# LLaVA-VL/LLaVA-Plus-Codebase

Hardware: NVIDIA H100
Metric: prefill+decode tokens/s (higher is better)
Workload: dtype bf16

## Files before the change

llava-plus-codebase_b200/csrc/decode_mega.cu:

```cuda
#include <limits.h>
#include <math.h>

#include "common.cuh"
#include "kernels.h"

namespace b2 {
namespace {

constexpr int MK_CONS_WARPS = 16;
constexpr int MK_CONS = MK_CONS_WARPS * 32;
constexpr int MK_PROD_WARPS = 4;
constexpr int MK_THREADS = MK_CONS + 32 * MK_PROD_WARPS;
constexpr int MK_D = 128;
constexpr int MK_U = 4;
constexpr int MK_KT = 2048;
constexpr int MK_ROW_PAD = 64;
constexpr int MK_ROW_STRIDE = MK_KT * 2 + MK_ROW_PAD;
constexpr int MK_TILE_BYTES = 8 * MK_ROW_STRIDE;
constexpr int MK_MAXNB = 32;
constexpr int MK_MAXL = 48;
constexpr int MK_MAX_STAGES = 12;

__device__ __forceinline__ void unpack8(const uint4& u, float (&f)[8]) {
    f[0] = bf16_lo(u.x); f[1] = bf16_hi(u.x); f[2] = bf16_lo(u.y); f[3] = bf16_hi(u.y);
    f[4] = bf16_lo(u.z); f[5] = bf16_hi(u.z); f[6] = bf16_lo(u.w); f[7] = bf16_hi(u.w);
}
__device__ __forceinline__ uint4 ldcg16(const void* p) { return __ldcg(reinterpret_cast<const uint4*>(p)); }

__device__ __forceinline__ void cons_sync() { asm volatile("bar.sync 1, %0;" ::"n"(MK_CONS) : "memory"); }

__device__ __forceinline__ void grid_sync(unsigned int* counter, unsigned int target) {
    cons_sync();
    if (threadIdx.x == 0) {
        asm volatile("red.release.gpu.global.add.u32 [%0], 1;" ::"l"(counter) : "memory");
        unsigned int cur, spins = 0;
        do {
            asm volatile("ld.acquire.gpu.global.u32 %0, [%1];" : "=r"(cur) : "l"(counter) : "memory");
            if (++spins > (1u << 26)) asm volatile("trap;");
        } while ((int)(cur - target) < 0);
    }
    cons_sync();
}

__device__ __forceinline__ void bulk_g2s(void* smem_dst, const void* gsrc, uint32_t bytes, uint64_t* bar) {
    asm volatile("cp.async.bulk.shared::cluster.global.mbarrier::complete_tx::bytes [%0], [%1], %2, [%3];" ::"r"(
                     smem_u32(smem_dst)),
                 "l"(gsrc), "r"(bytes), "r"(smem_u32(bar))
                 : "memory");
}

struct GemvCtx {
    const __nv_bfloat16* W;
    int K, act;
    int u_lo, nu;
    int nb;
    int nchunk;
};
struct PhaseIO {
    const __nv_bfloat16* xin;
    const __nv_bfloat16* gamma;
    const __nv_bfloat16* residual;
    void* out;
    int ld_out, out_fp32;
};

__device__ __forceinline__ int mk_phys_row(const GemvCtx& c, int rb, int g, bool& valid) {
    if (c.act == ACT_SWIGLU) {
        const int lc = rb * 4 + (g & 3);
        valid = lc < c.nu;
        const int ch = c.u_lo + lc;
        return (ch >> 6) * 128 + (ch & 63) + ((g >> 2) ? 64 : 0);
    }
    const int lr = rb * 8 + g;
    valid = lr < c.nu;
    return c.u_lo + lr;
}

__device__ __forceinline__ int mk_rows_in_block(const GemvCtx& c, int rb) {
    if (c.act == ACT_SWIGLU) return 2 * min(4, c.nu - rb * 4);
    return min(8, c.nu - rb * 8);
}

__device__ __forceinline__ bool mk_is_attention(const MegaParams& p, int ph) { return ph % 5 == 1 && ph < 5 * p.L; }

__device__ __forceinline__ PhaseIO mk_phase_io(const MegaParams& p, const MegaLayer* layers, int ph) {
    PhaseIO c;
    const int l = ph / 5, k = ph % 5;
    c.gamma = nullptr; c.residual = nullptr; c.out_fp32 = 0;
    if (l >= p.L) { c.xin = p.x; c.gamma = p.final_norm; c.out = p.logits; c.ld_out = p.V; c.out_fp32 = 1; }
    else if (k <= 1) { c.xin = p.x; c.gamma = layers[l].ln1; c.out = p.qkv; c.ld_out = 3 * p.h; }
    else if (k == 2) { c.xin = p.attn; c.residual = p.x; c.out = p.x; c.ld_out = p.h; }
    else if (k == 3) { c.xin = p.x; c.gamma = layers[l].ln2; c.out = p.act; c.ld_out = p.I; }
    else { c.xin = p.act; c.residual = p.x; c.out = p.x; c.ld_out = p.h; }
    return c;
}
__device__ __forceinline__ GemvCtx mk_phase_ctx(const MegaParams& p, const MegaLayer* layers, int ph) {
    GemvCtx c;
    const int l = ph / 5, k = ph % 5;
    int N;
    c.act = ACT_NONE;
    if (l >= p.L) { c.W = p.lm_head; N = p.V; c.K = p.h; }
    else if (k <= 1) { c.W = layers[l].wqkv; N = 3 * p.h; c.K = p.h; }
    else if (k == 2) { c.W = layers[l].wo; N = p.h; c.K = p.h; }
    else if (k == 3) { c.W = layers[l].wgu; N = 2 * p.I; c.K = p.h; c.act = ACT_SWIGLU; }
    else { c.W = layers[l].wd; N = p.h; c.K = p.I; }
    const long long units = c.act == ACT_SWIGLU ? (N >> 1) : N;
    c.u_lo = (int)((units * blockIdx.x) / gridDim.x);
    c.nu = (int)((units * (blockIdx.x + 1)) / gridDim.x) - c.u_lo;
    c.nb = c.act == ACT_SWIGLU ? (c.nu + 3) >> 2 : (c.nu + 7) >> 3;
    c.nchunk = (c.K + MK_KT - 1) / MK_KT;
    return c;
}

template <int NB>
__device__ __forceinline__ void mk_prologue(const PhaseIO& c, int K, int B, float eps, int tid, int lane, int warp,
                                            __nv_bfloat16* xs, float (*s_red)[NB], float* s_rstd,
                                            const __nv_bfloat16* gamma_smem) {
    const int nvec = K >> 3;
    float ss[NB];
#pragma unroll
    for (int b = 0; b < NB; ++b) ss[b] = 0.f;
    for (int i = tid; i < nvec; i += MK_CONS) {
#pragma unroll
        for (int b = 0; b < NB; ++b) {
            uint4 u = make_uint4(0, 0, 0, 0);
            if (b < B) u = ldcg16(c.xin + (size_t)b * K + i * 8);
            *reinterpret_cast<uint4*>(xs + (size_t)b * K + i * 8) = u;
            if (c.gamma != nullptr) {
                float f[8];
                unpack8(u, f);
#pragma unroll
                for (int e = 0; e < 8; ++e) ss[b] += f[e] * f[e];
            }
        }
    }
    if (c.gamma != nullptr) {
// ... 22 lines not shown
                const float rstd = s_rstd[b];
#pragma unroll
                for (int e = 0; e < 8; ++e) o[e] = gf[e] * round_bf16(f[e] * rstd);
                *px = make_uint4(pack_bf16(o[0], o[1]), pack_bf16(o[2], o[3]), pack_bf16(o[4], o[5]),
                                 pack_bf16(o[6], o[7]));
            }
        }
    }
    cons_sync();
}

__device__ __forceinline__ void mk_mma(float (&c)[4], uint32_t a0, uint32_t a2, uint32_t b0, uint32_t b1) {
    asm volatile(
        "mma.sync.aligned.m16n8k16.row.col.f32.bf16.bf16.f32 {%0,%1,%2,%3}, {%4,%5,%6,%7}, {%8,%9}, {%0,%1,%2,%3};"
        : "+f"(c[0]), "+f"(c[1]), "+f"(c[2]), "+f"(c[3])
        : "r"(a0), "r"(0u), "r"(a2), "r"(0u), "r"(b0), "r"(b1));
}

template <int NB>
__device__ __forceinline__ float mk_row_value(const float* s_gpart, int rb, int b, int r) {
    float v = 0.f;
#pragma unroll
    for (int ww = 0; ww < MK_CONS_WARPS; ++ww) v += s_gpart[(((size_t)ww * MK_MAXNB + rb) * NB + b) * 8 + r];
    return v;
}

template <int NB>
__device__ __forceinline__ void mk_epilogue(const MegaParams& p, const MegaLayer* layers, int ph, const GemvCtx& c,
                                            int B, int tid, const float* s_gpart, float res_pref, bool have_res_pref) {
    const PhaseIO io = mk_phase_io(p, layers, ph);
    if (c.act == ACT_SWIGLU) {
        const int nch = c.nu;
        for (int idx = tid; idx < nch * B; idx += MK_CONS) {
            const int b = idx / nch, r = idx - b * nch;
            const int rb = r >> 2, q = r & 3;
            const float gt = mk_row_value<NB>(s_gpart, rb, b, q);
            const float up = mk_row_value<NB>(s_gpart, rb, b, q + 4);
            reinterpret_cast<__nv_bfloat16*>(io.out)[(size_t)b * io.ld_out + (size_t)c.u_lo + r] =
                __float2bfloat16_rn(gt / (1.0f + __expf(-gt)) * up);
        }
    } else {
        const int nr = c.nu;
        for (int idx = tid; idx < nr * B; idx += MK_CONS) {
            const int b = idx / nr, r = idx - b * nr;
            float y = mk_row_value<NB>(s_gpart, r >> 3, b, r & 7);
            const size_t o = (size_t)b * io.ld_out + (size_t)c.u_lo + r;
            if (io.residual != nullptr) y += have_res_pref ? res_pref : __bfloat162float(__ldcg(io.residual + o));
            if (io.out_fp32) reinterpret_cast<float*>(io.out)[o] = y;
            else reinterpret_cast<__nv_bfloat16*>(io.out)[o] = __float2bfloat16_rn(y);
        }
    }
}

__device__ __forceinline__ void mk_attention(const MegaParams& p, const MegaLayer& Lw, int tid, int lane, int warp,
                                             float (*s_part)[MK_D + 2], int* s_flag, const float* s_cos,
                                             const float* s_sin) {
    const int h = p.h, H = p.H;
    const int pairs = p.B * H;
    const int grid = gridDim.x;
    const int G = pairs <= grid ? grid / pairs : 1;
    const int hw = lane >> 4, c = lane & 15;
    const int split = pairs <= grid ? (int)blockIdx.x % G : 0;
    for (int pair = pairs <= grid ? (int)blockIdx.x / G : (int)blockIdx.x; pair < pairs;
         pair += (pairs <= grid ? pairs : grid)) {
        const int head = pair % H, b = pair / H;
        const int pos = p.cur_len[b];
        const int total = pos + 1;
        const int cchunk = (total + G - 1) / G;
        const int cb = split * cchunk;
        const int ce = min(cb + cchunk, total);
        const int wchunk = (max(ce - cb, 0) + MK_CONS_WARPS - 1) / MK_CONS_WARPS;
        const int k_begin = cb + warp * wchunk;
        const int k_end = min(k_begin + wchunk, ce);
        const __nv_bfloat16* qrow = p.qkv + (size_t)b * 3 * h + head * MK_D;
        float qreg[8], knew[8], vnew[8];
        {
            float qa[8], qb[8], ka[8], kb[8];
            unpack8(ldcg16(qrow + c * 8), qa);
            unpack8(ldcg16(qrow + (c ^ 8) * 8), qb);
            unpack8(ldcg16(qrow + h + c * 8), ka);
            unpack8(ldcg16(qrow + h + (c ^ 8) * 8), kb);
            unpack8(ldcg16(qrow + 2 * h + c * 8), vnew);
            const float sign = (c < 8) ? -1.f : 1.f;
#pragma unroll
            for (int e = 0; e < 8; ++e) {
                const int i = ((c & 7) * 8 + e);
                const float cbf = s_cos[b * 64 + i], sbf = s_sin[b * 64 + i];
                qreg[e] = round_bf16(round_bf16(qa[e] * cbf) + round_bf16(sign * qb[e] * sbf));
                knew[e] = round_bf16(round_bf16(ka[e] * cbf) + round_bf16(sign * kb[e] * sbf));
            }
        }
        const size_t cbase = ((size_t)b * H + head) * p.Smax * MK_D;
        if (pos >= k_begin && pos < k_end && hw == 0) {
            *reinterpret_cast<uint4*>(Lw.kcache + cbase + (size_t)pos * MK_D + c * 8) =
                make_uint4(pack_bf16(knew[0], knew[1]), pack_bf16(knew[2], knew[3]),
                           pack_bf16(knew[4], knew[5]), pack_bf16(knew[6], knew[7]));
            *reinterpret_cast<uint4*>(Lw.vcache + cbase + (size_t)pos * MK_D + c * 8) =
                make_uint4(pack_bf16(vnew[0], vnew[1]), pack_bf16(vnew[2], vnew[3]),
                           pack_bf16(vnew[4], vnew[5]), pack_bf16(vnew[6], vnew[7]));
        }
        float m_run = -INFINITY, l_run = 0.f, av[8];
#pragma unroll
        for (int e = 0; e < 8; ++e) av[e] = 0.f;
        const __nv_bfloat16* kb_ = Lw.kcache + cbase + c * 8;
        const __nv_bfloat16* vb_ = Lw.vcache + cbase + c * 8;
        for (int kbase = k_begin; kbase < k_end; kbase += 2 * MK_U) {
            uint4 kraw[MK_U], vraw[MK_U];
#pragma unroll
            for (int u = 0; u < MK_U; ++u) {
                const int key = kbase + hw + 2 * u;
                if (key < k_end && key != pos) {
                    kraw[u] = ld_stream_16(kb_ + (size_t)key * MK_D);
                    vraw[u] = ld_stream_16(vb_ + (size_t)key * MK_D);
                } else {
                    kraw[u] = make_uint4(0, 0, 0, 0);
                    vraw[u] = make_uint4(0, 0, 0, 0);
                }
            }
#pragma unroll
            for (int u = 0; u < MK_U; ++u) {
                const int key = kbase + hw + 2 * u;
                float kf[8], vf[8];
                unpack8(kraw[u], kf);
                unpack8(vraw[u], vf);
                if (key == pos) {
#pragma unroll
                    for (int e = 0; e < 8; ++e) { kf[e] = knew[e]; vf[e] = vnew[e]; }
// ... 30 lines not shown
            }
            l_run = l_run * w_s + l_o * w_o;
            m_run = m_c;
        }
        if (hw == 0) {
#pragma unroll
            for (int e = 0; e < 8; ++e) s_part[warp][c * 8 + e] = av[e];
            if (c == 0) { s_part[warp][MK_D] = m_run; s_part[warp][MK_D + 1] = l_run; }
        }
        cons_sync();
        float m_cta = -INFINITY, l_cta = 0.f, o_cta = 0.f;
        if (tid < MK_D) {
#pragma unroll
            for (int i = 0; i < MK_CONS_WARPS; ++i) m_cta = fmaxf(m_cta, s_part[i][MK_D]);
#pragma unroll
            for (int i = 0; i < MK_CONS_WARPS; ++i) {
                const float ms = s_part[i][MK_D];
                const float wgt = (ms == -INFINITY) ? 0.f : exp2f(ms - m_cta);
                l_cta += s_part[i][MK_D + 1] * wgt;
                o_cta += s_part[i][tid] * wgt;
            }
        }
        if (G == 1) {
            if (tid < MK_D) p.attn[(size_t)b * h + head * MK_D + tid] = __float2bfloat16_rn(o_cta / l_cta);
        } else {
            float* part = p.attn_partial + ((size_t)pair * G + split) * (MK_D + 2);
            if (tid < MK_D) {
                part[tid] = o_cta;
                if (tid == 0) { part[MK_D] = m_cta; part[MK_D + 1] = l_cta; }
            }
            __threadfence();
            cons_sync();
            if (tid == 0) *s_flag = (atomicAdd(&p.attn_counters[pair], 1) == G - 1) ? 1 : 0;
            cons_sync();
            if (*s_flag) {
                __threadfence();
                if (tid < MK_D) {
                    const float* pb = p.attn_partial + (size_t)pair * G * (MK_D + 2);
                    float m_all = -INFINITY;
                    for (int sidx = 0; sidx < G; ++sidx) m_all = fmaxf(m_all, __ldcg(pb + (size_t)sidx * (MK_D + 2) + MK_D));
                    float l_all = 0.f, o_all = 0.f;
                    for (int sidx = 0; sidx < G; ++sidx) {
                        const float ms = __ldcg(pb + (size_t)sidx * (MK_D + 2) + MK_D);
                        const float wgt = (ms == -INFINITY) ? 0.f : exp2f(ms - m_all);
                        l_all += __ldcg(pb + (size_t)sidx * (MK_D + 2) + MK_D + 1) * wgt;
                        o_all += __ldcg(pb + (size_t)sidx * (MK_D + 2) + tid) * wgt;
                    }
                    p.attn[(size_t)b * h + head * MK_D + tid] = __float2bfloat16_rn(o_all / l_all);
                    if (tid == 0) p.attn_counters[pair] = 0;
                }
            }
        }
        cons_sync();
    }
}

struct TileCursor {
    GemvCtx c;
    int ph, rb, kc;
    uint32_t tile;
    bool valid;
};
__device__ __forceinline__ void cursor_seek(TileCursor& t, const MegaParams& p, const MegaLayer* layers, int n_phases) {
    while (t.ph < n_phases) {
        if (!mk_is_attention(p, t.ph)) {
            t.c = mk_phase_ctx(p, layers, t.ph);
            if (t.c.nb > 0) { t.rb = 0; t.kc = 0; t.valid = true; return; }
        }
        ++t.ph;
    }
    t.valid = false;
}
__device__ __forceinline__ void cursor_begin(TileCursor& t, const MegaParams& p, const MegaLayer* layers, int n_phases) {
    t.ph = 0; t.tile = 0; t.rb = 0; t.kc = 0;
    cursor_seek(t, p, layers, n_phases);
}
__device__ __forceinline__ void cursor_next(TileCursor& t, const MegaParams& p, const MegaLayer* layers, int n_phases) {
    ++t.tile;
    if (++t.kc < t.c.nchunk) return;
    t.kc = 0;
    if (++t.rb < t.c.nb) return;
    ++t.ph;
    cursor_seek(t, p, layers, n_phases);
}
template <int NB>
__global__ void __launch_bounds__(MK_THREADS, 1) decode_mega_kernel(MegaParams p, int n_stages) {
    extern __shared__ __align__(128) uint8_t mk_smem[];
    uint8_t* ring = mk_smem;
    __nv_bfloat16* xs = reinterpret_cast<__nv_bfloat16*>(ring + (size_t)n_stages * MK_TILE_BYTES);
    float* s_gpart = reinterpret_cast<float*>(reinterpret_cast<uint8_t*>(xs) + (size_t)NB * (p.h > p.I ? p.h : p.I) * 2);
    uint64_t* full_bar = reinterpret_cast<uint64_t*>(s_gpart + (size_t)MK_CONS_WARPS * MK_MAXNB * NB * 8);
    uint64_t* empty_bar = full_bar + MK_MAX_STAGES;
    __shared__ float s_red[MK_CONS_WARPS][NB];
    __shared__ float s_rstd[NB];
    __shared__ float s_av[MK_CONS_WARPS];
    __shared__ int s_ai[MK_CONS_WARPS];
    __shared__ float s_part[MK_CONS_WARPS][MK_D + 2];
    __shared__ int s_flag;
    __shared__ float s_cos[NB * 64], s_sin[NB * 64];
    __shared__ __align__(16) MegaLayer s_layers[MK_MAXL];

    const int tid = threadIdx.x, lane = tid & 31, warp = tid >> 5;
    const int B = p.B;
    const int n_phases = 5 * p.L + 1;

    {
// ... 12 lines not shown

    if (warp >= MK_CONS_WARPS) {
        const uint32_t pw = (uint32_t)(warp - MK_CONS_WARPS);
        TileCursor cp;
        cursor_begin(cp, p, s_layers, n_phases);
        while (cp.valid) {
            if (cp.tile % (uint32_t)MK_PROD_WARPS == pw) {
                const uint32_t stage = cp.tile % (uint32_t)n_stages;
                const uint32_t parity = (cp.tile / (uint32_t)n_stages) & 1u;
                const uint32_t row_bytes = (uint32_t)min(MK_KT, cp.c.K - cp.kc * MK_KT) * 2u;
                if (lane == 0) {
                    mbar_wait(&empty_bar[stage], parity ^ 1u);
                    mbar_arrive_expect_tx(&full_bar[stage], (uint32_t)mk_rows_in_block(cp.c, cp.rb) * row_bytes);
                }
                __syncwarp();
                bool row_valid;
                const int prow = mk_phys_row(cp.c, cp.rb, lane & 7, row_valid);
                if (lane < 8 && row_valid)
                    bulk_g2s(ring + (size_t)stage * MK_TILE_BYTES + (size_t)lane * MK_ROW_STRIDE,
                             cp.c.W + (size_t)prow * cp.c.K + (size_t)cp.kc * MK_KT, row_bytes, &full_bar[stage]);
            }
            cursor_next(cp, p, s_layers, n_phases);
        }
        return;
    }

    for (int i = tid; i < B * 64; i += MK_CONS) {
        const int b = i >> 6, f = i & 63;
        const float inv_freq = exp2f(-(2.0f * f / MK_D) * log2f(p.theta));
        float sv, cv;
        sincosf((float)p.cur_len[b] * inv_freq, &sv, &cv);
        s_cos[i] = round_bf16(cv);
        s_sin[i] = round_bf16(sv);
    }
    if (blockIdx.x < B) {
        int t = p.tok[blockIdx.x];
        t = t < 0 ? 0 : (t >= p.V ? p.V - 1 : t);
        const uint4* src = reinterpret_cast<const uint4*>(p.embed + (size_t)t * p.h);
        uint4* dst = reinterpret_cast<uint4*>(p.x + (size_t)blockIdx.x * p.h);
        for (int i = tid; i < p.h / 8; i += MK_CONS) dst[i] = src[i];
    }
    __nv_bfloat16* gsm = xs + (size_t)NB * p.h;
    const bool gsm_fits = (size_t)(NB + 1) * p.h <= (size_t)NB * (p.h > p.I ? p.h : p.I);
    auto gamma_prefetch = [&](int ph) -> bool {
        if (!gsm_fits || ph >= n_phases || mk_is_attention(p, ph)) return false;
        const PhaseIO io = mk_phase_io(p, s_layers, ph);
        if (io.gamma == nullptr) return false;
        for (int i = tid; i < (p.h >> 3); i += MK_CONS)
            asm volatile("cp.async.cg.shared.global [%0], [%1], 16;" ::"r"(smem_u32(gsm + i * 8)), "l"(io.gamma + i * 8) : "memory");
        asm volatile("cp.async.commit_group;" ::: "memory");
        return true;
    };
    bool gsm_ok = gamma_prefetch(0);
    unsigned int bar_target = p.bar_base + gridDim.x;
    grid_sync(p.bar_count, bar_target);

    const bool tracing = p.trace != nullptr && blockIdx.x == 0 && tid == 0;
    const int g = lane >> 2, t4 = lane & 3;
    uint32_t tile = 0;
#pragma unroll 1
    for (int ph = 0; ph < n_phases; ++ph) {
        if (tracing) p.trace[ph * 4 + 0] = clock64();
        if (mk_is_attention(p, ph)) {
            mk_attention(p, s_layers[ph / 5], tid, lane, warp, s_part, &s_flag, s_cos, s_sin);
        } else {
            const GemvCtx c = mk_phase_ctx(p, s_layers, ph);
            const PhaseIO io = mk_phase_io(p, s_layers, ph);
            const bool have_res = io.residual != nullptr && c.nu * B <= MK_CONS;
            float res_pref = 0.f;
            if (have_res && tid < c.nu * B) {
                const int b = tid / c.nu, r = tid - b * c.nu;
                res_pref = __bfloat162float(__ldcg(io.residual + (size_t)b * io.ld_out + (size_t)c.u_lo + r));
            }
            mk_prologue<NB>(io, c.K, B, p.eps, tid, lane, warp, xs, s_red, s_rstd, gsm_ok ? gsm : nullptr);
            if (tracing) p.trace[ph * 4 + 1] = clock64();
#pragma unroll 1
            for (int rb = 0; rb < c.nb; ++rb) {
                float acc[4] = {0.f, 0.f, 0.f, 0.f}, acc2[4] = {0.f, 0.f, 0.f, 0.f};
#pragma unroll 1
                for (int kc = 0; kc < c.nchunk; ++kc, ++tile) {
                    const uint32_t stage = tile % (uint32_t)n_stages;
                    const uint32_t parity = (tile / (uint32_t)n_stages) & 1u;
                    const int nk32 = min(MK_KT, c.K - kc * MK_KT) >> 5;
                    mbar_wait(&full_bar[stage], parity);
                    const uint8_t* trow = ring + (size_t)stage * MK_TILE_BYTES + (size_t)g * MK_ROW_STRIDE + t4 * 16;
                    const __nv_bfloat16* xrow = xs + (size_t)g * c.K + (size_t)kc * MK_KT + t4 * 8;
#pragma unroll 4
                    for (int k32 = warp; k32 < nk32; k32 += MK_CONS_WARPS) {
                        const uint4 wv = *reinterpret_cast<const uint4*>(trow + k32 * 64);
                        uint4 xv = make_uint4(0, 0, 0, 0);
                        if (g < B) xv = *reinterpret_cast<const uint4*>(xrow + k32 * 32);
                        mk_mma(acc, xv.x, xv.y, wv.x, wv.y);
                        mk_mma(acc2, xv.z, xv.w, wv.z, wv.w);
                    }
                    __syncwarp();
                    if (lane == 0) mbar_arrive(&empty_bar[stage]);
                }
                if (g < NB)
                    *reinterpret_cast<float2*>(s_gpart + (((size_t)warp * MK_MAXNB + rb) * NB + g) * 8 + t4 * 2) =
                        make_float2(acc[0] + acc2[0], acc[1] + acc2[1]);
            }
            cons_sync();
            if (tracing) p.trace[ph * 4 + 2] = clock64();
            mk_epilogue<NB>(p, s_layers, ph, c, B, tid, s_gpart, res_pref, have_res);
        }
        if (tracing) p.trace[ph * 4 + 3] = clock64();
        gsm_ok = gamma_prefetch(ph + 1);
        bar_target += gridDim.x;
        grid_sync(p.bar_count, bar_target);
    }
    if (tracing) p.trace[n_phases * 4] = clock64();

    if (blockIdx.x < B) {
        const int b = blockIdx.x;
        const float* row = p.logits + (size_t)b * p.V;
        float best = -INFINITY;
        int bi = INT_MAX;
        for (int i = tid; i < p.V; i += MK_CONS) {
            const float v = __ldcg(row + i);
            if (v == v && (bi == INT_MAX || v > best)) { best = v; bi = i; }
        }
#pragma unroll
        for (int o = 16; o > 0; o >>= 1) {
            const float ov = __shfl_xor_sync(0xffffffffu, best, o);
            const int oi = __shfl_xor_sync(0xffffffffu, bi, o);
            if (ov > best || (ov == best && oi < bi)) { best = ov; bi = oi; }
        }
        if (lane == 0) { s_av[warp] = best; s_ai[warp] = bi; }
        cons_sync();
        if (warp == 0) {
            best = lane < MK_CONS_WARPS ? s_av[lane] : -INFINITY;
            bi = lane < MK_CONS_WARPS ? s_ai[lane] : INT_MAX;
#pragma unroll
            for (int o = 16; o > 0; o >>= 1) {
                const float ov = __shfl_xor_sync(0xffffffffu, best, o);
                const int oi = __shfl_xor_sync(0xffffffffu, bi, o);
                if (ov > best || (ov == best && oi < bi)) { best = ov; bi = oi; }
            }
            if (lane == 0) {
                const int tk = bi == INT_MAX ? 0 : bi;
                p.tok[b] = tk;
                p.out_tokens[(size_t)(*p.step_counter) * B + b] = tk;
                if (p.rows == nullptr || p.rows[b].active) p.cur_len[b] += 1;
                if (p.ring != nullptr) {
                    const int pub = p.sstate->pub_counter, tag0 = p.sstate->tag;
                    if (tag0 != 0) {
                        const int tag = 1 + (tag0 - 1 + pub / p.ring_cap) % 2047;
                        reinterpret_cast<volatile int32_t*>(p.ring)[(size_t)(pub % p.ring_cap) * B + b] = (tag << 20) | (tk & 0xFFFFF);
                        __threadfence_system();
                    }
                }
            }
        }
    }
    cons_sync();
    if (tid == 0) {
        __threadfence();
        if (atomicAdd(p.done_count, 1u) == gridDim.x - 1) {
            *p.done_count = 0u;
            *p.step_counter += 1;
            if (p.ring != nullptr) p.sstate->pub_counter += 1;
        }
    }
}

size_t mega_fixed_bytes(int NB, int h, int I) {
    return (size_t)NB * (h > I ? h : I) * 2 + (size_t)MK_CONS_WARPS * MK_MAXNB * NB * 8 * 4 + 2 * MK_MAX_STAGES * 8;
}
size_t mega_static_bytes(int NB) {
    return (size_t)(MK_CONS_WARPS + 1) * NB * 4 + MK_CONS_WARPS * (MK_D + 2 + 2) * 4 + NB * 512 +
           MK_MAXL * sizeof(MegaLayer) + 1024;
}
int mega_stages(int NB, int h, int I) {
    const long long avail = 227 * 1024 - (long long)mega_fixed_bytes(NB, h, I) - (long long)mega_static_bytes(NB);
    long long s = avail / MK_TILE_BYTES;
    return (int)(s > MK_MAX_STAGES ? MK_MAX_STAGES : s);
}

}

bool decode_mega_fits(int B, int h, int I) {
    if (B < 1 || B > 2) return false;
    return mega_stages(B, h, I) >= 4;
}

int decode_mega(const MegaParams& p, cudaStream_t stream) {
    B2_CHECK_ARG(p.B >= 1 && p.B <= 2, "decode_mega: batch must be 1..2");
    B2_CHECK_ARG(p.L <= MK_MAXL, "decode_mega: %d layers exceed the shared layer table (%d)", p.L, MK_MAXL);
    B2_CHECK_ARG(p.h % 256 == 0 && p.I % 256 == 0 && p.V % 8 == 0 && p.h / p.H == MK_D,
                 "decode_mega: unsupported dims h=%d I=%d V=%d H=%d", p.h, p.I, p.V, p.H);
    {
        const int grid = num_sms();
        const int nmax = p.V > 3 * p.h ? (p.V > 2 * p.I ? p.V : 2 * p.I) : (3 * p.h > 2 * p.I ? 3 * p.h : 2 * p.I);
        B2_CHECK_ARG((nmax / 8 + grid - 1) / grid + 1 <= MK_MAXNB,
                     "decode_mega: %d output rows per CTA exceed the shared-memory block table", nmax / grid);
    }
    const int NB = p.B;
    const int stages = mega_stages(NB, p.h, p.I);
    B2_CHECK_ARG(stages >= 4, "decode_mega: shared memory too small for the weight ring (B=%d h=%d I=%d)", p.B, p.h, p.I);
    const size_t smem = (size_t)stages * MK_TILE_BYTES + mega_fixed_bytes(NB, p.h, p.I);
    void* fn = NB == 1 ? (void*)decode_mega_kernel<1> : (void*)decode_mega_kernel<2>;
    static size_t attr_smem[3] = {0, 0, 0};
    if (smem > attr_smem[NB]) {
        B2_CUDA_CHECK(cudaFuncSetAttribute(fn, cudaFuncAttributeMaxDynamicSharedMemorySize, (int)smem));
        attr_smem[NB] = smem;
    }
    MegaParams pp = p;
    int n_stages = stages;
    void* args[] = {&pp, &n_stages};
    B2_CUDA_CHECK(cudaLaunchCooperativeKernel(fn, dim3(num_sms()), dim3(MK_THREADS), args, smem, stream));
    B2_LAUNCH_CHECK();
    return 0;
}

}
```

llava-plus-codebase_b200/csrc/kernels.h:

```cpp
#pragma once
#include <cuda_bf16.h>
#include <cuda_runtime.h>
#include <stdint.h>

namespace b2 {

enum { ACT_NONE = 0, ACT_QUICK_GELU = 1, ACT_GELU_ERF = 2, ACT_SWIGLU = 3, ACT_ROPE_QKV = 4 };

struct RopeQkv {
    const void* table = nullptr;
    void* kcache = nullptr;
    void* vcache = nullptr;
    int S = 0, H = 0, Smax = 0;
    const int32_t* pos0 = nullptr;
};
enum { DT_BF16 = 0, DT_F16 = 1, DT_F32 = 2 };

int num_sms();

struct GemmArgs {
    const void* A = nullptr; int lda = 0;
    const void* W = nullptr; int ldw = 0;
    const void* bias = nullptr;
    const void* residual = nullptr; int ld_res = 0;
// ... 80 lines not shown
int rope_table_build(void* table, int Smax, int D, float theta, cudaStream_t stream);
int rope_kv_write(void* qkv, void* kcache, void* vcache, int B, int S, int H, int D, int Smax, float theta,
                  cudaStream_t stream, const int32_t* pos0 = nullptr);

struct DecodeAttnArgs {
    const void* qkv = nullptr;
    void* kcache = nullptr; void* vcache = nullptr;
    float* kscale = nullptr; float* vscale = nullptr;
    const int32_t* cur_len = nullptr;
    void* out = nullptr;
    float* partial = nullptr;
    int32_t* counters = nullptr;
    int B = 0, H = 0, D = 128, Smax = 0, nsplit = 1;
    float theta = 10000.f, scale = 1.f;
    int R = 1;
};
int decode_attn_ctas_per_sm();
int decode_attn_bf16(const DecodeAttnArgs& a, cudaStream_t stream);
int decode_attn_mq_ctas_per_sm();
size_t decode_attn_mq_scratch_bytes(int B, int H, int nsplit);
int decode_attn_mq_bf16(const DecodeAttnArgs& a, cudaStream_t stream);
constexpr int kPrefixGroupRows = 16;
struct PrefixGroup {
    int32_t src_slot, prefix_len, n_rows;
    int32_t rows[kPrefixGroupRows];
};
int decode_attn_shared_ctas_per_sm();
size_t decode_attn_shared_scratch_bytes(int B, int H, int nsplit);
int decode_attn_shared_bf16(const DecodeAttnArgs& a, const PrefixGroup* groups, const int32_t* row_prefix, int G,
                            cudaStream_t stream);
int decode_attn_e4m3_ctas_per_sm();
int decode_attn_e4m3(const DecodeAttnArgs& a, cudaStream_t stream);
int kv_quantize_e4m3(const void* ksrc, const void* vsrc, void* k8, void* v8, float* kscale, float* vscale,
                     const int32_t* seq_lens, int B, int S, int H, int D, int Smax, cudaStream_t stream,
                     const int32_t* pos0 = nullptr, int S_src = 0);
int kv_dequantize_e4m3(const void* k8, const void* v8, const float* kscale, const float* vscale, const int32_t* pos0, void* kdst,
                       void* vdst, int B, int H, int Smax, int S_dst, cudaStream_t stream);

struct MegaLayer {
    const __nv_bfloat16 *ln1, *wqkv, *wo, *ln2, *wgu, *wd;
    __nv_bfloat16 *kcache, *vcache;
};
struct MegaParams {
    const MegaLayer* layers = nullptr;
    int L = 0, h = 0, I = 0, H = 0, V = 0, B = 0, Smax = 0, nsplit = 1;
    const __nv_bfloat16 *embed = nullptr, *final_norm = nullptr, *lm_head = nullptr;
    int32_t *tok = nullptr, *cur_len = nullptr, *out_tokens = nullptr, *step_counter = nullptr;
    __nv_bfloat16 *x = nullptr, *qkv = nullptr, *attn = nullptr, *act = nullptr;
    float* logits = nullptr;
    float* attn_partial = nullptr;
    int32_t* attn_counters = nullptr;
    unsigned int *bar_count = nullptr, *done_count = nullptr;
    unsigned int bar_base = 0;
    float eps = 1e-5f, theta = 10000.f, scale_log2 = 1.f;
    long long* trace = nullptr;
    struct SampleState* sstate = nullptr;
    int32_t* ring = nullptr;
    int ring_cap = 0;
    const struct RowState* rows = nullptr;
};
int decode_mega(const MegaParams& p, cudaStream_t stream);
bool decode_mega_fits(int B, int h, int I);

struct SampleState {
    int do_sample;
    float temperature, top_p;
    int top_k;
    unsigned long long seed;
    int tag;
    int pub_counter;
    unsigned int done;
    int per_row;
    float* out_scores;
    float* out_logits;
    int out_cap;
};
struct RowState {
    int active;
    int do_sample; float temperature, top_p; int top_k;
    unsigned long long seed;
    int index;
};
constexpr int kProcMaxEos = 8;
struct ProcRow {
    int on;
    float penalty;
    int ngram;
    int min_gen;
    int n_eos;
    int eos[kProcMaxEos];
    int prompt_len;
    int hist_len;
};
struct ProcState {
    ProcRow* rows;
    int32_t* hist;
    uint32_t* bits;
    int cap, words;
};
constexpr int kSpecMaxRows = 16;
struct SpecState {
    int K;
    int ngram;
    int max_new;
    int n_eos;
    int eos[kProcMaxEos];
    int prompt_len;
    int hist_len;
    int draft_len;
    int32_t rows[kSpecMaxRows];
    int steps, drafted, accepted;
    int retired;
    int32_t sel[kSpecMaxRows];
    int* mirror;
// ... 78 lines not shown
```

llava-plus-codebase_b200/csrc/model.cu:

```cuda
#include <cuda_fp16.h>
#include <limits.h>
#include <stdarg.h>
#include <stdio.h>
#include <stdlib.h>
#include <string.h>
#include <time.h>

#include <array>
#include <atomic>
#include <utility>
#include <mutex>
#include <string>
#include <vector>

#include "../../include/b2llava.h"
#include "common.cuh"
#include "kernels.h"

namespace b2 {

static thread_local char g_err[1024] = {0};
unsigned long long g_launch_count = 0;

void set_error(const char* fmt, ...) {
// ... 57 lines not shown
}
}

using namespace b2;

struct b2_model {
    b2_model_desc d;
    int device = 0;
    std::mutex mu;
    bool finalized = false;
    int P = 0, T = 0, kpad = 0, vit_live = 0, vit_hd = 64, hd = 128;
    DevBuf patch_w, cls, pos, pre_g, pre_b;
    std::vector<VitLayer> vit;
    DevBuf p0_w, p0_b, p2_w, p2_b;
    DevBuf embed, final_norm;
    Linear head;
    std::vector<LlamaLayer> ll;
    int* err_host = nullptr;
    int* err_dev = nullptr;
    cudaEvent_t ws_event = nullptr;
    cudaStream_t ws_stream = nullptr;
    bool ws_valid = false;
    DevBuf v_col, v_patch, v_hidden, v_xn, v_qkv, v_attn, v_mlp, v_feats, p_mid, p_done;
    DevBuf x, xn, qkv, attn, act, last_idx, xlast, logits, splice_idx;
    DevBuf chunk_pos;
    DevBuf enc_pixels, enc_out;
    std::vector<cudaGraphExec_t> enc_graph;
    std::vector<char> enc_warm;
    cudaStream_t enc_stream = nullptr;
    cudaEvent_t enc_fork = nullptr, enc_join = nullptr;
    int enc_launches = 0;
    bool fp8_decode = false;
    DevBuf xq8, xscale;
    DevBuf kstage, vstage;
    bool nf4 = false;
    DevBuf nf4_scratch;
    std::atomic<int> kv_live{0};
};

struct b2_kv {
    b2_model* m = nullptr;
    int max_batch = 0, max_seq = 0;
    int dtype = B2_KV_BF16;
    int pitch = 0;
    DevBuf k, v;
    DevBuf kscale, vscale;
    DevBuf len_dev, tok, step_counter, out_tokens, attn_partial, attn_counters;
    DevBuf sk_partial, sk_counters;
    std::vector<int32_t> len_host;
    int out_capacity = 0;
    cudaGraphExec_t graph = nullptr;
    int graph_B = 0;
    int graph_launches = 0;
    unsigned int mega_bar_base = 0;
    DevBuf mega_layers, mega_sync;
    DevBuf rope_tab;
    cudaStream_t own_stream = nullptr;
    cudaEvent_t ev_fork = nullptr, ev_join = nullptr;
    int warm_B = 0;
    DevBuf sstate;
    SampleState samp_host = {};
    bool samp_valid = false;
    int32_t* ring_host = nullptr;
    int32_t* ring_dev = nullptr;
    int ring_cap = 0;
    int epoch = 0;
    int stream_B = 0, stream_tag = 0, stream_scheduled = 0;
    float* next_scores = nullptr;
    float* next_logits = nullptr;
    int next_cap = 0;
    DevBuf rows_dev;
    std::vector<RowState> rows_host;
    DevBuf beam_in, beam_ws, beam_out;
    DevBuf proc_rows, proc_hist, proc_bits;
    std::vector<char> proc_on;
    bool any_proc() const { for (char c : proc_on) if (c) return true; return false; }
    DevBuf beam_proc_rows;
    bool beam_proc_on = false;
    DevBuf spec_state, spec_logits, spec_attn;
    int* spec_mirror = nullptr;
    int spec_nsplit = 0;
    int spec_R = 0;
    int spec_max_new = 0;
    int spec_queued = 0;
    int spec_len0 = 0;
    std::array<cudaGraphExec_t, kSpecMaxRows + 1> spec_graph{};
    std::array<int, kSpecMaxRows + 1> spec_launches{};
    std::array<char, kSpecMaxRows + 1> spec_warm{};
    DevBuf share_tab, share_attn;
    int share_G = 0;
    bool counted = false;
    bool e4m3() const { return dtype == B2_KV_E4M3; }
    size_t elem_bytes() const { return e4m3() ? 1 : 2; }
    size_t layer_rows() const { return (size_t)max_batch * m->d.heads * pitch; }
    size_t layer_stride() const { return layer_rows() * m->hd; }
    char* k_layer(int l) const { return k.as<char>() + (size_t)l * layer_stride() * elem_bytes(); }
    char* v_layer(int l) const { return v.as<char>() + (size_t)l * layer_stride() * elem_bytes(); }
};

namespace {

ProcState proc_state(const b2_kv* kv) {
    ProcState p = {};
    if (kv->proc_rows.p == nullptr) return p;
    p.rows = kv->proc_rows.as<ProcRow>(); p.hist = kv->proc_hist.as<int32_t>(); p.bits = kv->proc_bits.as<uint32_t>();
    p.cap = kv->max_seq + 1; p.words = (kv->m->d.vocab + 31) / 32;
    return p;
// ... 413 lines not shown
    B2_TRY(decode_linear(m, kv, plan.head, m->head, m->head.w.p, m->x.p, h, m->final_norm.p, false, m->logits.p, V, 1, B, V, h,
                         ACT_NONE, st));
    B2_TRY(sample_publish(m->logits.as<float>(), V, B, kv->sstate.as<SampleState>(), kv->rows_dev.as<RowState>(), kv->tok.as<int32_t>(),
                          kv->out_tokens.as<int32_t>(), kv->step_counter.as<int32_t>(), kv->len_dev.as<int32_t>(),
                          kv->ring_dev, kv->ring_cap, SP_SELECT | SP_WRITE_OUT | SP_BUMP, 0, proc_state(kv), nullptr, st));
    return 0;
}

int fork_stream(b2_kv* kv, cudaStream_t st, cudaStream_t* run) {
    if (st != nullptr && st != cudaStreamLegacy) { *run = st; return 0; }
    if (kv->own_stream == nullptr) {
        B2_CUDA_CHECK(cudaStreamCreateWithFlags(&kv->own_stream, cudaStreamNonBlocking));
        B2_CUDA_CHECK(cudaEventCreateWithFlags(&kv->ev_fork, cudaEventDisableTiming));
        B2_CUDA_CHECK(cudaEventCreateWithFlags(&kv->ev_join, cudaEventDisableTiming));
    }
    B2_CUDA_CHECK(cudaEventRecord(kv->ev_fork, st));
    B2_CUDA_CHECK(cudaStreamWaitEvent(kv->own_stream, kv->ev_fork, 0));
    *run = kv->own_stream;
    return 0;
}
int join_stream(b2_kv* kv, cudaStream_t st, cudaStream_t run) {
    if (run == st) return 0;
    B2_CUDA_CHECK(cudaEventRecord(kv->ev_join, run));
    B2_CUDA_CHECK(cudaStreamWaitEvent(st, kv->ev_join, 0));
    return 0;
}

bool use_mega(const b2_model* m, const b2_kv* kv, int B) {
    if (kv->e4m3()) return false;
    if (m->nf4) return false;
    if (!decode_mega_fits(B, m->d.hidden, m->d.inter) || m->d.layers > 48) return false;
    static int flag = -1;
    if (flag < 0) {
        const char* e = getenv("B2_DECODE_MEGA");
        flag = (e != nullptr && e[0] == '0') ? 0 : 1;
    }
    return flag == 1;
}

int decode_step_mega(b2_model* m, b2_kv* kv, int B, cudaStream_t st) {
    const b2_model_desc& d = m->d;
    MegaParams p;
    p.layers = kv->mega_layers.as<MegaLayer>();
    p.L = d.layers; p.h = d.hidden; p.I = d.inter; p.H = d.heads; p.V = d.vocab; p.B = B; p.Smax = kv->pitch;
    int ns = (num_sms() * 16) / (B * d.heads);
    p.nsplit = ns < 1 ? 1 : (ns > 64 ? 64 : ns);
    p.embed = m->embed.as<bf16>(); p.final_norm = m->final_norm.as<bf16>(); p.lm_head = m->head.w.as<bf16>();
    p.tok = kv->tok.as<int32_t>(); p.cur_len = kv->len_dev.as<int32_t>();
    p.out_tokens = kv->out_tokens.as<int32_t>(); p.step_counter = kv->step_counter.as<int32_t>();
    p.x = m->x.as<bf16>(); p.qkv = m->qkv.as<bf16>(); p.attn = m->attn.as<bf16>(); p.act = m->act.as<bf16>();
    p.logits = m->logits.as<float>();
    p.attn_partial = kv->attn_partial.as<float>(); p.attn_counters = kv->attn_counters.as<int32_t>();
    unsigned int* sync = kv->mega_sync.as<unsigned int>();
    p.bar_count = sync; p.done_count = sync + 2;
    p.bar_base = kv->mega_bar_base;
    kv->mega_bar_base += (unsigned int)(5 * d.layers + 2) * (unsigned int)num_sms();
    p.eps = d.rms_eps; p.theta = d.rope_theta;
    p.scale_log2 = (1.0f / sqrtf((float)m->hd)) * 1.4426950408889634f;
    const bool sampling = kv->samp_host.do_sample != 0 || kv->samp_host.per_row != 0 || kv->any_proc();
    if (!sampling && kv->samp_host.tag != 0) { p.sstate = kv->sstate.as<SampleState>(); p.ring = kv->ring_dev; p.ring_cap = kv->ring_cap; }
    if (kv->samp_host.per_row) p.rows = kv->rows_dev.as<RowState>();
    static int trace_mode = -1;
    if (trace_mode < 0) { const char* e = getenv("B2_MEGA_TRACE"); trace_mode = (e && e[0] != 0) ? 1 : 0; }
    if (trace_mode == 1) {
        static int steps_seen = 0;
        if (++steps_seen == 40) {
            const int n = (5 * d.layers + 2) * 4;
            DevBuf tb;
            B2_TRY(tb.alloc((size_t)n * 8));
            cudaMemset(tb.p, 0, (size_t)n * 8);
            p.trace = tb.as<long long>();
            int r = decode_mega(p, st);
            cudaStreamSynchronize(st);
            std::vector<long long> host(n);
            cudaMemcpy(host.data(), tb.p, (size_t)n * 8, cudaMemcpyDeviceToHost);
            FILE* f = fopen(getenv("B2_MEGA_TRACE"), "w");
            if (f) {
                for (int ph = 0; ph <= 5 * d.layers; ++ph)
                    fprintf(f, "%d %lld %lld %lld %lld %lld\n", ph, host[ph * 4], host[ph * 4 + 1], host[ph * 4 + 2],
                            host[ph * 4 + 3], host[(ph + 1) * 4]);
                fclose(f);
            }
            tb.free();
            return r;
        }
    }
    B2_TRY(decode_mega(p, st));
    if (!sampling && p.ring != nullptr && kv->samp_host.out_cap > 0)
        B2_TRY(publish_rows(m->logits.as<float>(), d.vocab, B, kv->sstate.as<SampleState>(), st));
    if (sampling)
        B2_TRY(sample_publish(m->logits.as<float>(), d.vocab, B, kv->sstate.as<SampleState>(), kv->rows_dev.as<RowState>(), kv->tok.as<int32_t>(),
                              kv->out_tokens.as<int32_t>(), kv->step_counter.as<int32_t>(), kv->len_dev.as<int32_t>(),
                              kv->ring_dev, kv->ring_cap, SP_SELECT | SP_WRITE_OUT, -1, proc_state(kv), nullptr, st));
    return 0;
}

static void share_arm(b2_kv* kv, int G) {
    if (kv->share_G == G) return;
    if (kv->graph) { cudaGraphExecDestroy(kv->graph); kv->graph = nullptr; kv->graph_B = 0; }
    kv->warm_B = 0;
    kv->share_G = G;
}
int decode_step_run(b2_model* m, b2_kv* kv, int B, cudaStream_t st) {
    if (use_mega(m, kv, B)) return decode_step_mega(m, kv, B, st);
    if (kv->warm_B != B) {
        if (kv->graph) { cudaGraphExecDestroy(kv->graph); kv->graph = nullptr; kv->graph_B = 0; }
        B2_TRY(decode_step_launch(m, kv, B, st));
        kv->warm_B = B;
        return 0;
// ... 405 lines not shown
        for (const Linear* lin : L.linears()) n += lin->bytes();
    }
    return (int64_t)n;
}

int b2_kv_create(b2_model* m, int max_batch, int max_seq, b2_kv** out) {
    return b2_kv_create_ex(m, max_batch, max_seq, B2_KV_BF16, out);
}

int b2_kv_create_ex(b2_model* m, int max_batch, int max_seq, int kv_dtype, b2_kv** out) {
    B2_CHECK_ARG(m && out, "b2_kv_create: null argument");
    B2_CHECK_ARG(kv_dtype == B2_KV_BF16 || kv_dtype == B2_KV_E4M3, "b2_kv_create: unknown kv_dtype %d (B2_KV_BF16 = 0, B2_KV_E4M3 = 1)",
                 kv_dtype);
    B2_CHECK_ARG(max_batch >= 1 && max_batch <= m->d.max_batch, "b2_kv_create: max_batch %d exceeds model max_batch %d",
                 max_batch, m->d.max_batch);
    B2_CHECK_ARG(max_seq >= 1, "b2_kv_create: max_seq must be positive");
    std::lock_guard<std::mutex> lk(m->mu);
    DeviceGuard dg(m->device);
    b2_kv* kv = new b2_kv();
    kv->m = m;
    kv->max_batch = max_batch;
    kv->max_seq = max_seq;
    kv->dtype = kv_dtype;
    kv->pitch = kv->e4m3() ? (max_seq + 3) / 4 * 4 : max_seq;
    const size_t per = (size_t)m->d.layers * kv->layer_stride() * kv->elem_bytes();
    const size_t per_scale = kv->e4m3() ? (size_t)m->d.layers * kv->layer_rows() * sizeof(float) : 0;
    int r = 0;
    if (kv->e4m3() && m->kstage.p == nullptr) {
        const size_t stage = (size_t)m->d.max_batch * m->d.max_seq * m->d.hidden * 2;
        if ((r = m->kstage.alloc(stage)) != 0 || (r = m->vstage.alloc(stage)) != 0) {
            m->kstage.free();
            delete kv;
            return r;
        }
    }
    if ((r = kv->k.alloc(per)) != 0 || (r = kv->v.alloc(per)) != 0 ||
        (r = kv->kscale.alloc(per_scale)) != 0 || (r = kv->vscale.alloc(per_scale)) != 0 ||
        (r = kv->len_dev.alloc((size_t)max_batch * 4)) != 0 || (r = kv->tok.alloc((size_t)max_batch * 4)) != 0 ||
        (r = kv->step_counter.alloc(4)) != 0) {
        b2_kv_destroy(kv);
        return r;
    }
    kv->out_capacity = max_seq;
    const int max_split = 64;
    if (!m->nf4) {
        std::vector<MegaLayer> tbl(m->d.layers);
        for (int l = 0; l < m->d.layers; ++l) {
            LlamaLayer& L = m->ll[l];
            tbl[l].ln1 = L.ln1.as<bf16>(); tbl[l].wqkv = L.qkv.w.as<bf16>(); tbl[l].wo = L.o.w.as<bf16>();
            tbl[l].ln2 = L.ln2.as<bf16>(); tbl[l].wgu = L.gu.w.as<bf16>(); tbl[l].wd = L.d.w.as<bf16>();
            tbl[l].kcache = reinterpret_cast<bf16*>(kv->k_layer(l));
            tbl[l].vcache = reinterpret_cast<bf16*>(kv->v_layer(l));
        }
        if ((r = kv->mega_layers.alloc(tbl.size() * sizeof(MegaLayer))) != 0 || (r = kv->mega_sync.alloc(64)) != 0) {
            b2_kv_destroy(kv);
            return r;
        }
        cudaMemcpy(kv->mega_layers.p, tbl.data(), tbl.size() * sizeof(MegaLayer), cudaMemcpyHostToDevice);
        cudaMemset(kv->mega_sync.p, 0, 64);
    }
    if ((r = kv->out_tokens.alloc((size_t)kv->out_capacity * max_batch * 4)) != 0 ||
        (r = kv->attn_partial.alloc(((size_t)max_batch * m->d.heads * max_split + 1024) * (128 + 2) * 4)) != 0 ||
        (r = kv->attn_counters.alloc((size_t)max_batch * m->d.heads * 4)) != 0) {
        b2_kv_destroy(kv);
        return r;
    }
    if (max_batch >= 7 && max_batch <= 128) {
        size_t ws = 0;
        int nmax = 0;
        auto fit = [&](int N, int K) {
            const size_t b = gemm_skinny_workspace_bytes(max_batch, N, K);
            ws = b > ws ? b : ws;
            nmax = N > nmax ? N : nmax;
        };
        for (const LinearShape& sh : layer_shapes(m->d)) fit(sh.N, sh.K);
        fit(m->d.vocab, m->d.hidden);
        if ((r = kv->sk_partial.alloc(ws)) != 0 || (r = kv->sk_counters.alloc(gemm_skinny_counter_bytes(nmax))) != 0) {
            b2_kv_destroy(kv);
            return r;
        }
        cudaMemset(kv->sk_counters.p, 0, gemm_skinny_counter_bytes(nmax));
    }
    kv->ring_cap = max_seq;
    if ((r = kv->sstate.alloc(sizeof(SampleState))) != 0 || (r = kv->rows_dev.alloc((size_t)max_batch * sizeof(RowState))) != 0) {
        b2_kv_destroy(kv);
        return r;
    }
    cudaMemset(kv->sstate.p, 0, sizeof(SampleState));
    cudaMemset(kv->rows_dev.p, 0, (size_t)max_batch * sizeof(RowState));
    kv->rows_host.assign(max_batch, RowState{});
    if (cudaHostAlloc(reinterpret_cast<void**>(&kv->ring_host), (size_t)kv->ring_cap * max_batch * 4, cudaHostAllocMapped) != cudaSuccess ||
        cudaHostGetDevicePointer(reinterpret_cast<void**>(&kv->ring_dev), kv->ring_host, 0) != cudaSuccess) {
        set_error("b2_kv_create: cannot allocate the pinned token ring (%d x %d)", kv->ring_cap, max_batch);
        cudaGetLastError();
        b2_kv_destroy(kv);
        return -2;
    }
    memset(kv->ring_host, 0, (size_t)kv->ring_cap * max_batch * 4);
    cudaMemset(kv->k.p, 0, per);
    cudaMemset(kv->v.p, 0, per);
    if (per_scale) { cudaMemset(kv->kscale.p, 0, per_scale); cudaMemset(kv->vscale.p, 0, per_scale); }
    cudaMemset(kv->len_dev.p, 0, (size_t)max_batch * 4);
    cudaMemset(kv->tok.p, 0, (size_t)max_batch * 4);
    cudaMemset(kv->step_counter.p, 0, 4);
    cudaMemset(kv->attn_counters.p, 0, (size_t)max_batch * m->d.heads * 4);
    if ((r = kv->rope_tab.alloc((size_t)max_seq * (m->hd / 2) * sizeof(uint32_t))) != 0 ||
        (r = rope_table_build(kv->rope_tab.p, max_seq, m->hd, m->d.rope_theta, nullptr)) != 0) {
        b2_kv_destroy(kv);
        return r;
    }
    B2_CUDA_CHECK(cudaDeviceSynchronize());
    kv->len_host.assign(max_batch, 0);
// ... 1436 lines not shown
```

Measured before the change: 729.3.

## Replace grid barriers around attention with per-head dataflow counters in decode megakernel

The persistent decode megakernel no longer runs a full grid barrier after the QKV projection and after attention. Each CTA publishes how many QKV rows it finished into a per-head counter, and attention CTAs wait only on the head they need. After attention, CTAs wait on a merged-heads counter instead of the grid barrier. This cuts two grid-wide barriers per layer in exchange for more counter bookkeeping and epoch bases tracked on the host. The added row-to-head mapping and the B-scaled merge counts are fragile if batch size or grid size change between steps.

```diff
diff --git a/llava-plus-codebase_b200/csrc/decode_mega.cu b/llava-plus-codebase_b200/csrc/decode_mega.cu
--- a/llava-plus-codebase_b200/csrc/decode_mega.cu
+++ b/llava-plus-codebase_b200/csrc/decode_mega.cu
@@ -29,15 +29,22 @@
 
 __device__ __forceinline__ void cons_sync() { asm volatile("bar.sync 1, %0;" ::"n"(MK_CONS) : "memory"); }
 
+__device__ __forceinline__ void mk_publish(unsigned int* counter, unsigned int n) {
+    asm volatile("red.release.gpu.global.add.u32 [%0], %1;" ::"l"(counter), "r"(n) : "memory");
+}
+__device__ __forceinline__ void mk_wait_for(const unsigned int* counter, unsigned int target) {
+    unsigned int cur, spins = 0;
+    do {
+        asm volatile("ld.acquire.gpu.global.u32 %0, [%1];" : "=r"(cur) : "l"(counter) : "memory");
+        if (++spins > (1u << 26)) asm volatile("trap;");
+    } while ((int)(cur - target) < 0);
+}
+
 __device__ __forceinline__ void grid_sync(unsigned int* counter, unsigned int target) {
     cons_sync();
     if (threadIdx.x == 0) {
-        asm volatile("red.release.gpu.global.add.u32 [%0], 1;" ::"l"(counter) : "memory");
-        unsigned int cur, spins = 0;
-        do {
-            asm volatile("ld.acquire.gpu.global.u32 %0, [%1];" : "=r"(cur) : "l"(counter) : "memory");
-            if (++spins > (1u << 26)) asm volatile("trap;");
-        } while ((int)(cur - target) < 0);
+        mk_publish(counter, 1);
+        mk_wait_for(counter, target);
     }
     cons_sync();
 }
@@ -82,6 +89,7 @@
 }
 
 __device__ __forceinline__ bool mk_is_attention(const MegaParams& p, int ph) { return ph % 5 == 1 && ph < 5 * p.L; }
+__device__ __forceinline__ bool mk_is_qkv(const MegaParams& p, int ph) { return ph % 5 == 0 && ph < 5 * p.L; }
 
 __device__ __forceinline__ PhaseIO mk_phase_io(const MegaParams& p, const MegaLayer* layers, int ph) {
     PhaseIO c;
@@ -210,9 +218,9 @@
     }
 }
 
-__device__ __forceinline__ void mk_attention(const MegaParams& p, const MegaLayer& Lw, int tid, int lane, int warp,
-                                             float (*s_part)[MK_D + 2], int* s_flag, const float* s_cos,
-                                             const float* s_sin) {
+__device__ __forceinline__ void mk_attention(const MegaParams& p, const MegaLayer& Lw, unsigned int head_target, int tid,
+                                            int lane, int warp, float (*s_part)[MK_D + 2], int* s_flag,
+                                            const float* s_cos, const float* s_sin) {
     const int h = p.h, H = p.H;
     const int pairs = p.B * H;
     const int grid = gridDim.x;
@@ -231,6 +239,8 @@
         const int k_begin = cb + warp * wchunk;
         const int k_end = min(k_begin + wchunk, ce);
         const __nv_bfloat16* qrow = p.qkv + (size_t)b * 3 * h + head * MK_D;
+        if (tid == 0) mk_wait_for(p.head_rows + head, head_target);
+        cons_sync();
         float qreg[8], knew[8], vnew[8];
         {
             float qa[8], qb[8], ka[8], kb[8];
@@ -367,6 +377,7 @@
             }
         }
         cons_sync();
+        if (tid == 0 && (G == 1 || *s_flag)) mk_publish(p.heads_merged, 1);
     }
 }
 
@@ -485,8 +496,7 @@
         return true;
     };
     bool gsm_ok = gamma_prefetch(0);
-    unsigned int bar_target = p.bar_base + gridDim.x;
-    grid_sync(p.bar_count, bar_target);
+    grid_sync(p.bar_count, p.bar_base + gridDim.x);
 
     const bool tracing = p.trace != nullptr && blockIdx.x == 0 && tid == 0;
     const int g = lane >> 2, t4 = lane & 3;
@@ -495,7 +505,8 @@
     for (int ph = 0; ph < n_phases; ++ph) {
         if (tracing) p.trace[ph * 4 + 0] = clock64();
         if (mk_is_attention(p, ph)) {
-            mk_attention(p, s_layers[ph / 5], tid, lane, warp, s_part, &s_flag, s_cos, s_sin);
+            mk_attention(p, s_layers[ph / 5], p.head_base + 3u * MK_D * (unsigned int)(ph / 5 + 1), tid, lane, warp,
+                         s_part, &s_flag, s_cos, s_sin);
         } else {
             const GemvCtx c = mk_phase_ctx(p, s_layers, ph);
             const PhaseIO io = mk_phase_io(p, s_layers, ph);
@@ -539,8 +550,22 @@
         }
         if (tracing) p.trace[ph * 4 + 3] = clock64();
         gsm_ok = gamma_prefetch(ph + 1);
-        bar_target += gridDim.x;
-        grid_sync(p.bar_count, bar_target);
+        if (mk_is_qkv(p, ph)) {
+            cons_sync();
+            if (tid < MK_MAXNB * 8 / MK_D + 1) {
+                const long long units = 3 * p.h;
+                const int lo = (int)((units * blockIdx.x) / gridDim.x), hi = (int)((units * (blockIdx.x + 1)) / gridDim.x);
+                const int blk = lo / MK_D + tid;
+                const int n = min(hi, (blk + 1) * MK_D) - max(lo, blk * MK_D);
+                if (n > 0) mk_publish(p.head_rows + blk % p.H, (unsigned int)n);
+            }
+        } else if (mk_is_attention(p, ph)) {
+            if (tid == 0) mk_wait_for(p.heads_merged, p.merge_base + (unsigned int)(B * p.H) * (unsigned int)(ph / 5 + 1));
+            cons_sync();
+        } else {
+            const int l = ph / 5, nbar = ph < 5 * p.L ? 1 + 3 * l + ph % 5 - 1 : 2 + 3 * p.L;
+            grid_sync(p.bar_count, p.bar_base + (unsigned int)nbar * gridDim.x);
+        }
     }
     if (tracing) p.trace[n_phases * 4] = clock64();
 
@@ -627,6 +652,7 @@
         const int nmax = p.V > 3 * p.h ? (p.V > 2 * p.I ? p.V : 2 * p.I) : (3 * p.h > 2 * p.I ? 3 * p.h : 2 * p.I);
         B2_CHECK_ARG((nmax / 8 + grid - 1) / grid + 1 <= MK_MAXNB,
                      "decode_mega: %d output rows per CTA exceed the shared-memory block table", nmax / grid);
+        B2_CHECK_ARG(3 * p.h >= grid, "decode_mega: %d QKV rows for %d CTAs", 3 * p.h, grid);
     }
     const int NB = p.B;
     const int stages = mega_stages(NB, p.h, p.I);
diff --git a/llava-plus-codebase_b200/csrc/kernels.h b/llava-plus-codebase_b200/csrc/kernels.h
--- a/llava-plus-codebase_b200/csrc/kernels.h
+++ b/llava-plus-codebase_b200/csrc/kernels.h
@@ -156,6 +156,8 @@
     int32_t* attn_counters = nullptr;
     unsigned int *bar_count = nullptr, *done_count = nullptr;
     unsigned int bar_base = 0;
+    unsigned int *head_rows = nullptr, *heads_merged = nullptr;
+    unsigned int head_base = 0, merge_base = 0;
     float eps = 1e-5f, theta = 10000.f, scale_log2 = 1.f;
     long long* trace = nullptr;
     struct SampleState* sstate = nullptr;
@@ -164,6 +166,7 @@
     const struct RowState* rows = nullptr;
 };
 int decode_mega(const MegaParams& p, cudaStream_t stream);
+inline size_t mega_sync_bytes(int H) { return (16 + (size_t)H) * 4; }
 bool decode_mega_fits(int B, int h, int I);
 
 struct SampleState {
diff --git a/llava-plus-codebase_b200/csrc/model.cu b/llava-plus-codebase_b200/csrc/model.cu
--- a/llava-plus-codebase_b200/csrc/model.cu
+++ b/llava-plus-codebase_b200/csrc/model.cu
@@ -133,7 +133,7 @@
     cudaGraphExec_t graph = nullptr;
     int graph_B = 0;
     int graph_launches = 0;
-    unsigned int mega_bar_base = 0;
+    unsigned int mega_bar_base = 0, mega_head_base = 0, mega_merge_base = 0;
     DevBuf mega_layers, mega_sync;
     DevBuf rope_tab;
     cudaStream_t own_stream = nullptr;
@@ -653,9 +653,13 @@
     p.logits = m->logits.as<float>();
     p.attn_partial = kv->attn_partial.as<float>(); p.attn_counters = kv->attn_counters.as<int32_t>();
     unsigned int* sync = kv->mega_sync.as<unsigned int>();
-    p.bar_count = sync; p.done_count = sync + 2;
+    p.bar_count = sync; p.done_count = sync + 2; p.heads_merged = sync + 3; p.head_rows = sync + 16;
     p.bar_base = kv->mega_bar_base;
-    kv->mega_bar_base += (unsigned int)(5 * d.layers + 2) * (unsigned int)num_sms();
+    p.head_base = kv->mega_head_base;
+    p.merge_base = kv->mega_merge_base;
+    kv->mega_bar_base += (unsigned int)(3 * d.layers + 2) * (unsigned int)num_sms();
+    kv->mega_head_base += (unsigned int)(3 * 128 * d.layers);
+    kv->mega_merge_base += (unsigned int)(B * d.heads * d.layers);
     p.eps = d.rms_eps; p.theta = d.rope_theta;
     p.scale_log2 = (1.0f / sqrtf((float)m->hd)) * 1.4426950408889634f;
     const bool sampling = kv->samp_host.do_sample != 0 || kv->samp_host.per_row != 0 || kv->any_proc();
@@ -1167,12 +1171,13 @@
             tbl[l].kcache = reinterpret_cast<bf16*>(kv->k_layer(l));
             tbl[l].vcache = reinterpret_cast<bf16*>(kv->v_layer(l));
         }
-        if ((r = kv->mega_layers.alloc(tbl.size() * sizeof(MegaLayer))) != 0 || (r = kv->mega_sync.alloc(64)) != 0) {
+        if ((r = kv->mega_layers.alloc(tbl.size() * sizeof(MegaLayer))) != 0 ||
+            (r = kv->mega_sync.alloc(mega_sync_bytes(m->d.heads))) != 0) {
             b2_kv_destroy(kv);
             return r;
         }
         cudaMemcpy(kv->mega_layers.p, tbl.data(), tbl.size() * sizeof(MegaLayer), cudaMemcpyHostToDevice);
-        cudaMemset(kv->mega_sync.p, 0, 64);
+        cudaMemset(kv->mega_sync.p, 0, mega_sync_bytes(m->d.heads));
     }
     if ((r = kv->out_tokens.alloc((size_t)kv->out_capacity * max_batch * 4)) != 0 ||
         (r = kv->attn_partial.alloc(((size_t)max_batch * m->d.heads * max_split + 1024) * (128 + 2) * 4)) != 0 ||
```

Measured after the change: 731.8, median of 6. No clear change (+0.3%).
